# wayveai/fiery

Hardware: NVIDIA H100
Metric: camera->BEV lift frames/sec (6-cam 224x480 -> 200x200) (higher is better)
Workload: dtype f32

## Files before the change

fiery_b200/csrc/common.cuh:

```cuda
#pragma once
#include <cuda.h>
#include <cuda_runtime.h>
#include <cuda_fp16.h>
#include <stdint.h>
#include <stdio.h>
#include <stdlib.h>
#include "../../include/fiery_b200.h"

namespace fiery {

int set_error(int code, const char* fmt, ...);

#define FIERY_CUDA_CHECK(expr)                                                                              \
    do {                                                                                                    \
        cudaError_t _e = (expr);                                                                            \
        if (_e != cudaSuccess)                                                                              \
            return ::fiery::set_error(FIERY_E_CUDA, "%s failed: %s (%s:%d)", #expr, cudaGetErrorString(_e), \
                                      __FILE__, __LINE__);                                                  \
    } while (0)

#define FIERY_REQUIRE(cond, ...)                                             \
    do {                                                                     \
        if (!(cond)) return ::fiery::set_error(FIERY_E_INVALID, __VA_ARGS__); \
    } while (0)
// ... 26 lines not shown
        "mbarrier.try_wait.parity.shared::cta.b64 p, [%1], %2;\n\t"
        "selp.u32 %0, 1, 0, p;\n\t}"
        : "=r"(ok)
        : "r"(smem_addr(bar)), "r"(parity)
        : "memory");
    return ok != 0;
}

__device__ __forceinline__ void mbar_wait(uint64_t* bar, uint32_t parity) {
    uint32_t spins = 0;
    while (!mbar_try_wait(bar, parity)) {
        if (++spins > (1u << 24)) __trap();
    }
}

__device__ __forceinline__ void bulk_load_1d(void* dst, const void* src, uint32_t bytes, uint64_t* bar) {
    asm volatile("cp.async.bulk.shared::cluster.global.mbarrier::complete_tx::bytes [%0], [%1], %2, [%3];"
                 ::"r"(smem_addr(dst)), "l"(src), "r"(bytes), "r"(smem_addr(bar)) : "memory");
}

__device__ __forceinline__ void tma_load_3d(void* dst, const CUtensorMap* map, uint64_t* bar, int c0, int c1, int c2) {
    asm volatile(
        "cp.async.bulk.tensor.3d.shared::cluster.global.mbarrier::complete_tx::bytes [%0], [%1, {%3, %4, %5}], [%2];"
        ::"r"(smem_addr(dst)), "l"(reinterpret_cast<uint64_t>(map)), "r"(smem_addr(bar)), "r"(c0), "r"(c1), "r"(c2)
        : "memory");
}

__device__ __forceinline__ void tma_load_4d(void* dst, const CUtensorMap* map, uint64_t* bar, int c0, int c1, int c2, int c3) {
    asm volatile(
        "cp.async.bulk.tensor.4d.shared::cluster.global.mbarrier::complete_tx::bytes [%0], [%1, {%3, %4, %5, %6}], [%2];"
        ::"r"(smem_addr(dst)), "l"(reinterpret_cast<uint64_t>(map)), "r"(smem_addr(bar)), "r"(c0), "r"(c1), "r"(c2), "r"(c3)
        : "memory");
}

__device__ __forceinline__ void tma_store_4d(const CUtensorMap* map, const void* src, int c0, int c1, int c2, int c3) {
    asm volatile("cp.async.bulk.tensor.4d.global.shared::cta.bulk_group [%0, {%2, %3, %4, %5}], [%1];"
                 ::"l"(reinterpret_cast<uint64_t>(map)), "r"(smem_addr(src)), "r"(c0), "r"(c1), "r"(c2), "r"(c3)
                 : "memory");
}

__device__ __forceinline__ void tma_store_commit_and_wait() {
    asm volatile("cp.async.bulk.commit_group;" ::: "memory");
    asm volatile("cp.async.bulk.wait_group.read 0;" ::: "memory");
}

__device__ __forceinline__ void tma_prefetch_desc(const CUtensorMap* map) {
// ... 31 lines not shown
```

fiery_b200/csrc/lift_fwd.cu:

```cuda
#include <atomic>
#include <mutex>

#include "lift_plan.cuh"
#include "warp_sample.cuh"

namespace fiery {

constexpr int FIN_THREADS = 256;
__global__ void __launch_bounds__(FIN_THREADS)
finalize_nchw_kernel(float* __restrict__ accum, unsigned char* __restrict__ flags, float* __restrict__ bev,
                     long long pillars, int blocks_per_frame, int clear_marks) {
    constexpr int C = 64;
    const int frame = blockIdx.x / blocks_per_frame;
    const long long pl = static_cast<long long>(blockIdx.x % blocks_per_frame) * FIN_THREADS + threadIdx.x;
    if (pl >= pillars) return;
    unsigned char* f = flags + static_cast<size_t>(frame) * pillars + pl;
    float4 v[C / 4];
    if (*f) {
        float4* row = reinterpret_cast<float4*>(accum + (static_cast<size_t>(frame) * pillars + pl) * C);
#pragma unroll
        for (int q = 0; q < C / 4; ++q) v[q] = row[q];
#pragma unroll
        for (int q = 0; q < C / 4; ++q) row[q] = make_float4(0.f, 0.f, 0.f, 0.f);
        if (clear_marks) *f = 0;
// ... 2 lines not shown
        for (int q = 0; q < C / 4; ++q) v[q] = make_float4(0.f, 0.f, 0.f, 0.f);
    }
    float* dst = bev + static_cast<size_t>(frame) * C * pillars + pl;
#pragma unroll
    for (int q = 0; q < C / 4; ++q) {
        dst[static_cast<size_t>(4 * q + 0) * pillars] = v[q].x;
        dst[static_cast<size_t>(4 * q + 1) * pillars] = v[q].y;
        dst[static_cast<size_t>(4 * q + 2) * pillars] = v[q].z;
        dst[static_cast<size_t>(4 * q + 3) * pillars] = v[q].w;
    }
}

constexpr int FT_P = 64;
constexpr int FT_THREADS = 256;

__device__ __forceinline__ void bulk_store_1d(void* dst, const void* src, uint32_t bytes) {
    asm volatile("cp.async.bulk.global.shared::cta.bulk_group [%0], [%1], %2;" ::"l"(dst), "r"(smem_addr(src)), "r"(bytes) : "memory");
}
__device__ __forceinline__ void mbar_arrive(uint64_t* bar) {
    asm volatile("mbarrier.arrive.shared::cta.b64 _, [%0];" ::"r"(smem_addr(bar)) : "memory");
}
__device__ __forceinline__ void tma_store_3d(const CUtensorMap* map, const void* src, int c0, int c1, int c2) {
    asm volatile("cp.async.bulk.tensor.3d.global.shared::cta.bulk_group [%0, {%2, %3, %4}], [%1];"
                 ::"l"(reinterpret_cast<uint64_t>(map)), "r"(smem_addr(src)), "r"(c0), "r"(c1), "r"(c2) : "memory");
}

__global__ void __launch_bounds__(FT_THREADS)
finalize_tma_kernel(const __grid_constant__ CUtensorMap bev_map, float* __restrict__ accum, unsigned char* __restrict__ touched,
                    long long pillars, int tiles_per_frame, int frame_out0, int clear_marks) {
    constexpr int C = 64;
    __shared__ __align__(128) float s_in[FT_P * C];
    __shared__ __align__(128) float s_out[C * FT_P];
    __shared__ __align__(16) float s_zero[C];
    __shared__ __align__(8) uint64_t bar;
    __shared__ unsigned char s_flag[FT_P];
    const int tid = threadIdx.x;
    const int frame = blockIdx.x / tiles_per_frame;
    const long long p0 = static_cast<long long>(blockIdx.x % tiles_per_frame) * FT_P;
    if (tid == 0) {
        tma_prefetch_desc(&bev_map);
        mbar_init(&bar, FT_P);
        fence_mbar_init();
    }
    if (tid >= FT_THREADS - C) s_zero[tid - (FT_THREADS - C)] = 0.f;
    __syncthreads();
    float* row = nullptr;
    unsigned char* mark = nullptr;
    if (tid < FT_P) {
        const long long p = p0 + tid;
        unsigned char f = 0;
        if (p < pillars) {
            mark = touched + static_cast<size_t>(frame) * pillars + p;
            f = *mark;
        }
        s_flag[tid] = f;
        if (f) {
            row = accum + (static_cast<size_t>(frame) * pillars + p) * C;
            mbar_arrive_expect_tx(&bar, C * 4);
            bulk_load_1d(s_in + tid * C, row, C * 4, &bar);
        } else {
            mbar_arrive(&bar);
        }
    }
    __syncthreads();
    mbar_wait(&bar, 0);
    {
        const int lane = tid & 31, w = tid >> 5;
        const int pl = (w & 1) * 32 + lane;
        const int chunk0 = ((w >> 1) & 1) * 8;
        const int i0 = (w >> 2) * 4;
        const bool have = s_flag[pl] != 0;
        const float4* src = reinterpret_cast<const float4*>(s_in + pl * C);
        float* dst = s_out + pl;
        const int l7 = lane & 7;
#pragma unroll
        for (int ii = 0; ii < 4; ++ii) {
            const int chunk = chunk0 + ((i0 + ii) ^ l7);
            float4 v = make_float4(0.f, 0.f, 0.f, 0.f);
            if (have) v = src[chunk];
            float* d = dst + chunk * (4 * FT_P);
            d[0] = v.x; d[FT_P] = v.y; d[2 * FT_P] = v.z; d[3 * FT_P] = v.w;
        }
    }
    fence_proxy_async();
    __syncthreads();
    if (tid == 0) tma_store_3d(&bev_map, s_out, static_cast<int>(p0), 0, frame_out0 + frame);
    if (row) {
        bulk_store_1d(row, s_zero, C * 4);
        if (clear_marks) *mark = 0;
    }
    if (tid == 0 || row) tma_store_commit_and_wait();
}

constexpr int FW_P = 64;
constexpr int FW_THREADS = 256;
__global__ void __launch_bounds__(FW_THREADS)
finalize_warp_kernel(const float* __restrict__ accum, const unsigned char* __restrict__ touched, float* __restrict__ bev,
                     long long pillars, int H, int W, int tiles_per_frame, int frame_out0, const float* __restrict__ theta,
                     const unsigned char* __restrict__ copy_mask) {
    constexpr int C = 64;
    __shared__ float s_out[C][FW_P + 1];
    const int tid = threadIdx.x, lane = tid & 31, warp = tid >> 5;
    const int frame = blockIdx.x / tiles_per_frame;
// ... 25 lines not shown
                    b[k] = __ldg(row + 8 + l);
                }
            }
        }
        float4 ra, rb;
#define FIERY_BLEND(f) \
        ra.f = fmaf(w[3], a[3].f, fmaf(w[2], a[2].f, fmaf(w[1], a[1].f, w[0] * a[0].f))); \
        rb.f = fmaf(w[3], b[3].f, fmaf(w[2], b[2].f, fmaf(w[1], b[1].f, w[0] * b[0].f)));
        FIERY_BLEND(x) FIERY_BLEND(y) FIERY_BLEND(z) FIERY_BLEND(w)
#undef FIERY_BLEND
        s_out[4 * l + 0][pxl] = ra.x; s_out[4 * l + 1][pxl] = ra.y; s_out[4 * l + 2][pxl] = ra.z; s_out[4 * l + 3][pxl] = ra.w;
        s_out[32 + 4 * l + 0][pxl] = rb.x; s_out[32 + 4 * l + 1][pxl] = rb.y; s_out[32 + 4 * l + 2][pxl] = rb.z; s_out[32 + 4 * l + 3][pxl] = rb.w;
    }
    __syncthreads();
    float* dst = bev + static_cast<size_t>(gframe) * C * pillars + p0;
#pragma unroll
    for (int cc = 0; cc < C / (FW_THREADS / 32); ++cc) {
        const int c = warp * (C / (FW_THREADS / 32)) + cc;
#pragma unroll
        for (int half = 0; half < 2; ++half) {
            const int px = half * 32 + lane;
            if (p0 + px < pillars) __stcs(dst + static_cast<size_t>(c) * pillars + px, s_out[c][px]);
        }
    }
}

__global__ void __launch_bounds__(256)
clear_touched_kernel(float* __restrict__ accum, unsigned char* __restrict__ touched, long long n_pillars, int clear_marks) {
    const long long p = static_cast<long long>(blockIdx.x) * blockDim.x + threadIdx.x;
    const int lane = threadIdx.x & 31;
    const unsigned char f = p < n_pillars ? touched[p] : 0;
    unsigned m = __ballot_sync(0xffffffffu, f != 0);
    const long long base = p - lane;
    while (m) {
        const int i = __ffs(m) - 1;
        m &= m - 1;
        reinterpret_cast<float2*>(accum + static_cast<size_t>(base + i) * 64)[lane] = make_float2(0.f, 0.f);
    }
    if (f && clear_marks) touched[p] = 0;
}

__global__ void point_indices_kernel(const LiftParams P, int64_t* __restrict__ idx_out, uint8_t* __restrict__ valid_out,
                                     int32_t* __restrict__ pillar_out, long long n_points_total) {
    const long long gid = static_cast<long long>(blockIdx.x) * blockDim.x + threadIdx.x;
    if (gid >= n_points_total) return;
    const int w = static_cast<int>(gid % P.ww);
    long long r = gid / P.ww;
    const int h = static_cast<int>(r % P.hh); r /= P.hh;
    const int d = static_cast<int>(r % P.D); r /= P.D;
    const int cam_flat = static_cast<int>(r);
    CameraTransform T;
    load_camera(P.calib_mode, P.calib_a, P.calib_b, cam_flat, T);
// ... 23 lines not shown
    for (int k = 0; k < 3; ++k) translation[i * 3 + k] = T.t[k];
}

static std::atomic<int> g_max_chunk_frames{0};
void lift_set_max_chunk_frames(int n) { g_max_chunk_frames.store(n > 0 ? n : 0); }

int lift_chunk_frames(const LiftParams& P) {
    const long long per_frame = P.pillars * P.C * 4 + P.pillars;
    long long c = (1ll << 30) / (per_frame > 0 ? per_frame : 1);
    const int forced = g_max_chunk_frames.load();
    if (forced > 0 && forced < c) c = forced;
    if (c > P.n_frames) c = P.n_frames;
    return static_cast<int>(c < 1 ? 1 : c);
}

size_t lift_scratch_bytes(const LiftParams& P) {
    if (P.bev_layout != FIERY_BEV_NCHW || P.n_frames <= 0) return 0;
    const size_t chunk = static_cast<size_t>(lift_chunk_frames(P));
    return chunk * P.pillars * P.C * 4 + ((chunk * P.pillars + 127) & ~static_cast<size_t>(127));
}

int launch_forward_cols(const LiftParams& P, const void* head, cudaStream_t stream);
int encode_bev_map(CUtensorMap* map, float* bev, long long pillars, int channels, int n_frames, int box_pillars);

constexpr int MAX_CHAINS = 4;
struct ChainResources {
    cudaStream_t side[MAX_CHAINS - 1] = {};
    cudaEvent_t fork = nullptr;
    cudaEvent_t done[MAX_CHAINS - 1] = {};
    bool ready = false;
};
static int chain_resources(ChainResources** out) {
    static thread_local ChainResources pool[16];
    int dev = 0;
    FIERY_CUDA_CHECK(cudaGetDevice(&dev));
    FIERY_REQUIRE(dev >= 0 && dev < 16, "device %d out of range for the chain resources", dev);
    ChainResources& r = pool[dev];
    if (!r.ready) {
        for (int i = 0; i < MAX_CHAINS - 1; ++i) {
            FIERY_CUDA_CHECK(cudaStreamCreateWithFlags(&r.side[i], cudaStreamNonBlocking));
            FIERY_CUDA_CHECK(cudaEventCreateWithFlags(&r.done[i], cudaEventDisableTiming));
        }
        FIERY_CUDA_CHECK(cudaEventCreateWithFlags(&r.fork, cudaEventDisableTiming));
        r.ready = true;
    }
    *out = &r;
    return FIERY_OK;
}

#ifdef FIERY_COLS_AB
static int g_max_chains = MAX_CHAINS;
static int g_chain_min_tiles = 132;
#else
constexpr int g_max_chains = MAX_CHAINS;
constexpr int g_chain_min_tiles = 132;
#endif
int lift_forward_groups(const LiftParams& P, int frames_in_chunk) {
    if (P.bev_layout == FIERY_BEV_NHWC) return 1;
    int groups = frames_in_chunk < g_max_chains ? frames_in_chunk : g_max_chains;
    const long long tiles_per_frame = static_cast<long long>(P.n_cameras) * P.n_wtiles;
    while (groups > 1 && (frames_in_chunk / groups) * tiles_per_frame < g_chain_min_tiles) --groups;
    return groups < 1 ? 1 : groups;
}

int lift_forward_launches(const LiftParams& P) {
    if (P.n_frames <= 0) return 0;
    const int per_group = 1 + (P.bev_layout == FIERY_BEV_NCHW ? 1 : 0);
    const int chunk = lift_chunk_frames(P);
    int n = 0;
    for (int f0 = 0; f0 < P.n_frames; f0 += chunk)
        n += per_group * lift_forward_groups(P, (P.n_frames - f0 < chunk) ? P.n_frames - f0 : chunk);
    return n;
}

static thread_local LaunchTimer* g_timer = nullptr;
void lift_set_timer(LaunchTimer* t) { g_timer = t; }
static inline void timer_begin(cudaStream_t st, int kind) {
// ... 16 lines not shown
    FIERY_REQUIRE(P.D >= 1 && P.D <= 48, "depth_bins=%d not supported by this build (1..48)", P.D);
    FIERY_REQUIRE(P.ww % 4 == 0, "feat_w=%d must be a multiple of 4 (TMA row pitch must be 16-byte aligned)", P.ww);
    FIERY_REQUIRE(P.hh <= PLAN_MAX_ROWS, "feat_h=%d not supported by this build (<= %d)", P.hh, PLAN_MAX_ROWS);
    const bool nchw = P.bev_layout == FIERY_BEV_NCHW;
    FIERY_REQUIRE(!warp_theta || nchw, "the warped lift writes the NCHW layout only");
    FIERY_REQUIRE(scratch != nullptr || !nchw, "NCHW output needs the zeroed scratch buffer of fiery_lift_scratch_bytes()");
    int rc = FIERY_OK;
    LiftParams Q = P;
    Q.head_f16 = head_dtype == FIERY_DTYPE_F16 ? head : nullptr;
#ifdef FIERY_COLS_AB
    if (const char* e = getenv("FIERY_CHAINS")) g_max_chains = atoi(e) < MAX_CHAINS ? atoi(e) : MAX_CHAINS;
    if (const char* e = getenv("FIERY_CHAIN_MIN_TILES")) g_chain_min_tiles = atoi(e);
#endif
    const int chunk = lift_chunk_frames(P);
    float* accum = static_cast<float*>(scratch);
    unsigned char* scratch_marks = nchw ? reinterpret_cast<unsigned char*>(accum + static_cast<size_t>(chunk) * P.pillars * P.C) : nullptr;
    const bool tma_pass = P.pillars % 4 == 0;
    CUtensorMap bev_map;
    if (nchw && tma_pass && !warp_theta) {
        rc = encode_bev_map(&bev_map, bev_out, P.pillars, P.C, P.n_frames, FT_P);
        if (rc != FIERY_OK) return rc;
    }
    ChainResources* res = nullptr;
    for (int f0 = 0; f0 < P.n_frames; f0 += chunk) {
        const int nf = (P.n_frames - f0 < chunk) ? P.n_frames - f0 : chunk;
        const int groups = lift_forward_groups(P, nf);
        cudaStream_t chain[MAX_CHAINS] = {stream};
        if (groups > 1) {
            if (!res) {
                rc = chain_resources(&res);
                if (rc != FIERY_OK) return rc;
            }
            for (int g = 1; g < groups; ++g) chain[g] = res->side[g - 1];
            FIERY_CUDA_CHECK(cudaEventRecord(res->fork, stream));
        }
        for (int g = 0; g < groups; ++g) {
            const int s0 = static_cast<int>(static_cast<long long>(nf) * g / groups);
            const int s1 = static_cast<int>(static_cast<long long>(nf) * (g + 1) / groups);
            cudaStream_t st = chain[g];
            if (g > 0) FIERY_CUDA_CHECK(cudaStreamWaitEvent(st, res->fork, 0));
            Q.frame0 = f0 + s0;
            Q.n_frames = s1 - s0;
            unsigned char* marks = nullptr;
            if (plan) {
                const PlanView v = plan_view(plan, P.n_frames, P.n_cameras, P.n_wtiles, P.pillars, Q.frame0);
                Q.plan_tiles = v.tiles;
                Q.touched = nullptr;
                marks = const_cast<unsigned char*>(v.touched);
            } else {
                Q.plan_tiles = nullptr;
                marks = nchw ? scratch_marks + static_cast<size_t>(s0) * P.pillars : nullptr;
                Q.touched = marks;
            }
            Q.accum = nchw ? accum + static_cast<size_t>(s0) * P.pillars * P.C
                           : bev_out + static_cast<size_t>(Q.frame0) * P.pillars * P.C;
            timer_begin(st, 1);
            rc = launch_forward_cols(Q, head, st);
            timer_end(st);
            if (rc != FIERY_OK) return rc;
            if (nchw) {
                timer_begin(st, 2);
                if (warp_theta) {
                    const int tpf = static_cast<int>((P.pillars + FW_P - 1) / FW_P);
                    finalize_warp_kernel<<<static_cast<unsigned>(tpf) * Q.n_frames, FW_THREADS, 0, st>>>(
                        Q.accum, marks, bev_out, P.pillars, P.grid.X, P.grid.Y, tpf, Q.frame0, warp_theta, warp_copy);
                    const long long n = P.pillars * Q.n_frames;
                    clear_touched_kernel<<<static_cast<unsigned>((n + 255) / 256), 256, 0, st>>>(Q.accum, marks, n, plan ? 0 : 1);
                } else if (tma_pass) {
                    const int tpf = static_cast<int>((P.pillars + FT_P - 1) / FT_P);
                    finalize_tma_kernel<<<static_cast<unsigned>(tpf) * Q.n_frames, FT_THREADS, 0, st>>>(bev_map, Q.accum, marks, P.pillars,
                                                                                                     tpf, Q.frame0, plan ? 0 : 1);
                } else {
                    const int bpf = static_cast<int>((P.pillars + FIN_THREADS - 1) / FIN_THREADS);
                    finalize_nchw_kernel<<<static_cast<unsigned>(bpf) * Q.n_frames, FIN_THREADS, 0, st>>>(
                        Q.accum, marks, bev_out + static_cast<size_t>(Q.frame0) * P.C * P.pillars, P.pillars, bpf, plan ? 0 : 1);
                }
                timer_end(st);
                FIERY_CUDA_CHECK(cudaGetLastError());
            }
            if (g > 0) {
                FIERY_CUDA_CHECK(cudaEventRecord(res->done[g - 1], st));
                FIERY_CUDA_CHECK(cudaStreamWaitEvent(stream, res->done[g - 1], 0));
            }
        }
    }
    return FIERY_OK;
}

int launch_point_indices(const LiftParams& P, int64_t* idx_out, uint8_t* valid_out, int32_t* pillar_out, cudaStream_t stream) {
    const long long total = static_cast<long long>(P.n_frames) * P.n_cameras * P.D * P.hh * P.ww;
    if (total == 0) return FIERY_OK;
    const int threads = 256;
    point_indices_kernel<<<static_cast<unsigned>((total + threads - 1) / threads), threads, 0, stream>>>(
        P, idx_out, valid_out, pillar_out, total);
    FIERY_CUDA_CHECK(cudaGetLastError());
    return FIERY_OK;
}
// ... 10 lines not shown
```

fiery_b200/csrc/lift_fwd_cols.cu:

```cuda
#include <string.h>

#include "lift_plan.cuh"

namespace fiery {

constexpr int COLS_DPAD = 48;
constexpr int COLS_NPAIR = COLS_DPAD * WT;
constexpr int COLS_EVS = 33;
constexpr int COLS_PLAN_STAGE = 4096;
constexpr int COLS_RUNS_STAGED = (COLS_PLAN_STAGE - PLAN_OFF_RUNS) / 4;

struct HeadMapsCols {
    CUtensorMap depth;
    CUtensorMap ctx;
};

struct ColsLayout {
    int hh, C;
    int off_bar, off_plan, off_ev, off_prob, off_ctx, off_pillar, total;
    __host__ __device__ ColsLayout(int hh_, int C_, int n_units) : hh(hh_), C(C_) {
        int o = 0;
        off_bar = o;    o += 16;
        off_plan = o;   o += COLS_PLAN_STAGE;
        off_ev = o;     o += n_units * COLS_EVS * 4;
        o = (o + 127) & ~127;
        off_prob = o;   o += hh * COLS_DPAD * WT * 4;
        o = (o + 127) & ~127;
        off_ctx = o;    o += hh * C * WT * 4;
        o = (o + 127) & ~127;
        off_pillar = o; o += hh * COLS_NPAIR * 4;
        total = o;
    }
};

__device__ __forceinline__ void tma_load_5d(void* dst, const CUtensorMap* map, uint64_t* bar, int c0, int c1, int c2, int c3, int c4) {
    asm volatile(
        "cp.async.bulk.tensor.5d.shared::cluster.global.mbarrier::complete_tx::bytes [%0], [%1, {%3, %4, %5, %6, %7}], [%2];"
        ::"r"(smem_addr(dst)), "l"(reinterpret_cast<uint64_t>(map)), "r"(smem_addr(bar)), "r"(c0), "r"(c1), "r"(c2), "r"(c3), "r"(c4)
        : "memory");
}

__device__ __forceinline__ void cp_async_8(void* dst, const void* src) {
    asm volatile("cp.async.ca.shared.global [%0], [%1], 8;" ::"r"(smem_addr(dst)), "l"(src) : "memory");
}

__device__ __forceinline__ void ffma2(unsigned long long& acc, unsigned long long a, unsigned long long b) {
    asm("{\n\t.reg .f32 a0, a1, b0, b1, c0, c1;\n\t"
        "mov.b64 {a0, a1}, %1;\n\tmov.b64 {b0, b1}, %2;\n\tmov.b64 {c0, c1}, %0;\n\t"
        "fma.rn.f32 c0, a0, b0, c0;\n\tfma.rn.f32 c1, a1, b1, c1;\n\t"
        "mov.b64 %0, {c0, c1};\n\t}" : "+l"(acc) : "l"(a), "l"(b));
}

template <int HALF>
// ... 194 lines not shown
                sum += x[k];
            }
            sum += __shfl_xor_sync(0xffffffffu, sum, 4);
            sum += __shfl_xor_sync(0xffffffffu, sum, 8);
            sum += __shfl_xor_sync(0xffffffffu, sum, 16);
            const float inv = __fdiv_rn(1.0f, sum);
#pragma unroll
            for (int k = 0; k < COLS_DPAD / 8; ++k) base[k * 8 * WT] = x[k] * inv;
        } else {
#pragma unroll
            for (int k = 0; k < COLS_DPAD / 8; ++k) base[k * 8 * WT] = (c8 + 8 * k < P.D) ? 1.0f : 0.f;
        }
    }
}

template <int CPL>
__device__ __forceinline__ void red_channels_if(char* dst, const float (&v)[CPL], unsigned bit) {
    if (CPL == 4)
        asm volatile("{\n\t.reg .pred p;\n\tsetp.ne.u32 p, %5, 0;\n\t@p red.global.add.v4.f32 [%0], {%1, %2, %3, %4};\n\t}"
                     :: "l"(dst), "f"(v[0]), "f"(v[1]), "f"(v[CPL > 2 ? 2 : 0]), "f"(v[CPL > 3 ? 3 : 0]), "r"(bit) : "memory");
    else
        asm volatile("{\n\t.reg .pred p;\n\tsetp.ne.u32 p, %3, 0;\n\t@p red.global.add.v2.f32 [%0], {%1, %2};\n\t}"
                     :: "l"(dst), "f"(v[0]), "f"(v[1]), "r"(bit) : "memory");
}

template <int CPL, int DD, int SD, int COL>
__device__ __forceinline__ void flush_slot(unsigned long long (&acc)[CPL][DD][2], unsigned mw, unsigned own, unsigned flush,
                                           const int* plp, char* out) {
    constexpr int j = SD * 4 + COL;
    if (mw & (1u << j)) {
        const unsigned pl = static_cast<unsigned>(plp[j]);
        float v[CPL];
#pragma unroll
        for (int k = 0; k < CPL; ++k) v[k] = __fadd_rn(half_of<COL & 1>(acc[k][SD][COL >> 1]), 0.0f);
        red_channels_if<CPL>(out + static_cast<size_t>(pl) * (64 * 4), v, flush & (1u << j));
        const unsigned keep = ((own >> j) & 1u) - 1u;
#pragma unroll
        for (int k = 0; k < CPL; ++k) clear_half<COL & 1>(acc[k][SD][COL >> 1], keep);
    }
}

template <int CPL, int DD, int SD>
__device__ __forceinline__ void flush_depth(unsigned long long (&acc)[CPL][DD][2], unsigned mw, unsigned own, unsigned flush,
                                            const int* plp, char* out) {
    if (mw & (0xfu << (4 * SD))) {
        flush_slot<CPL, DD, SD, 0>(acc, mw, own, flush, plp, out); flush_slot<CPL, DD, SD, 1>(acc, mw, own, flush, plp, out);
        flush_slot<CPL, DD, SD, 2>(acc, mw, own, flush, plp, out); flush_slot<CPL, DD, SD, 3>(acc, mw, own, flush, plp, out);
    }
    if constexpr (SD + 1 < DD) flush_depth<CPL, DD, SD + 1>(acc, mw, own, flush, plp, out);
}

template <int CPL, int DD, int MINB, int UNR = 2, bool HALF = false, bool PLANNED = false>
__global__ void __launch_bounds__((COLS_DPAD / DD) * (64 / CPL), MINB)
lift_forward_cols_kernel(const __grid_constant__ HeadMapsCols head_maps, const LiftParams P) {
    constexpr int LPU = 64 / CPL;
    constexpr int NU = COLS_DPAD / DD;
    constexpr int NT = NU * LPU;
    constexpr int SLOTS = 4 * DD;
    static_assert(COLS_DPAD % DD == 0 && SLOTS <= 16 && (LPU == 16 || LPU == 32), "unsupported unit shape");
    extern __shared__ __align__(128) unsigned char smem[];
    const ColsLayout L(P.hh, P.C, NU);
    const int wtile = blockIdx.x % P.n_wtiles;
    const int img_local = blockIdx.x / P.n_wtiles;
    const int img = P.frame0 * P.n_cameras + img_local;
    const int frame = img_local / P.n_cameras;
    const int w0 = wtile * WT;
    const int tid = threadIdx.x;
// ... 5 lines not shown
        if (PLANNED) mbar_init(bar + 1, 1);
        if (!HALF) mbar_init(bar, 1);
        fence_mbar_init();
        if (PLANNED) {
            mbar_arrive_expect_tx(bar + 1, COLS_PLAN_STAGE);
            bulk_load_1d(smem + L.off_plan, rec, COLS_PLAN_STAGE, bar + 1);
        }
    }
    if (HALF) {
        issue_half_tile<CPL, NT>(P, L, smem, img, w0);
    } else if (tid == 0) {
        tma_prefetch_desc(&head_maps.depth);
        tma_prefetch_desc(&head_maps.ctx);
        const uint32_t prob_bytes = P.use_depth ? static_cast<uint32_t>(hh * COLS_DPAD * WT * 4) : 0u;
        mbar_arrive_expect_tx(bar, prob_bytes + static_cast<uint32_t>(hh * L.C * WT * 4));
        if (P.use_depth) tma_load_4d(smem + L.off_prob, &head_maps.depth, bar, w0, 0, 0, img);
        tma_load_5d(smem + L.off_ctx, &head_maps.ctx, bar, w0, 0, 0, 0, img);
    }
    {
        unsigned* s_ev = reinterpret_cast<unsigned*>(smem + L.off_ev);
        for (int i = tid; i < NU * COLS_EVS; i += NT) s_ev[i] = 0u;
    }
    if (!PLANNED) {
        float* s_u = reinterpret_cast<float*>(smem + L.off_plan + GEO_OFF_U);
        float* s_v = reinterpret_cast<float*>(smem + L.off_plan + GEO_OFF_V);
        float* s_d = reinterpret_cast<float*>(smem + L.off_plan + GEO_OFF_D);
        if (tid < WT) s_u[tid] = (w0 + tid < P.ww) ? P.fu[w0 + tid] : 0.f;
        if (tid >= 32 && tid < 64) s_v[tid - 32] = P.fv[min(tid - 32, hh - 1)];
        if (tid >= 64 && tid < 64 + COLS_DPAD) s_d[tid - 64] = (tid - 64 < P.D) ? P.fd[tid - 64] : 0.f;
        if (tid == NT - 1) {
            CameraTransform T;
            load_camera(P.calib_mode, P.calib_a, P.calib_b, img, T);
// ... 13 lines not shown
        if (P.grid.pow2[0] && P.grid.pow2[1]) stage_geometry_cols<true, NT, DD>(P, L, smem, w0, touched);
        else stage_geometry_cols<false, NT, DD>(P, L, smem, w0, touched);
    }
    if (HALF) widen_half_tile<NT>(P, L, smem);
    else mbar_wait(bar, 0);
    softmax_cols<NT>(P, L, smem);
    __syncthreads();

    const int unit = tid / LPU;
    const int cl = tid % LPU;
    const float* pp = reinterpret_cast<const float*>(smem + L.off_prob) + unit * DD * WT;
    const float* cp = reinterpret_cast<const float*>(smem + L.off_ctx) + cl * WT;
    const int* plp = reinterpret_cast<const int*>(smem + L.off_pillar) + unit * SLOTS - COLS_NPAIR;
    char* out = reinterpret_cast<char*>(P.accum + static_cast<size_t>(frame) * P.pillars * P.C + cl * CPL);
    const unsigned* evp = reinterpret_cast<const unsigned*>(smem + L.off_ev) + unit * COLS_EVS + 1;

    unsigned long long acc[CPL][DD][2];
#pragma unroll
    for (int k = 0; k < CPL; ++k)
#pragma unroll
        for (int dd = 0; dd < DD; ++dd) acc[k][dd][0] = acc[k][dd][1] = 0ull;

    unsigned own = 0, flush = 0, mw = 0;
#pragma unroll UNR
    for (int h = 0; h < hh; ++h, pp += COLS_DPAD * WT, cp += 64 * WT, plp += COLS_NPAIR, ++evp) {
        const unsigned ev_next = *evp;
        if (mw) flush_depth<CPL, DD, 0>(acc, mw, own, flush, plp, out);
        ulonglong2 dv[DD];
#pragma unroll
        for (int dd = 0; dd < DD; ++dd) dv[dd] = *reinterpret_cast<const ulonglong2*>(pp + dd * WT);
#pragma unroll
        for (int k = 0; k < CPL; ++k) {
            const ulonglong2 c = *reinterpret_cast<const ulonglong2*>(cp + k * LPU * WT);
#pragma unroll
            for (int dd = 0; dd < DD; ++dd) {
                ffma2(acc[k][dd][0], dv[dd].x, c.x);
                ffma2(acc[k][dd][1], dv[dd].y, c.y);
            }
        }
        own = ev_next & ((1u << SLOTS) - 1u);
        flush = ev_next >> SLOTS;
        mw = LPU == 32 ? own : __reduce_or_sync(0xffffffffu, own);
    }
#pragma unroll
    for (int j = 0; j < SLOTS; ++j) {
        const int pl = plp[j];
        float v[CPL];
#pragma unroll
        for (int k = 0; k < CPL; ++k) {
            const unsigned long long a = acc[k][j >> 2][(j & 3) >> 1];
            v[k] = (j & 1) ? half_of<1>(a) : half_of<0>(a);
        }
        red_channels_if<CPL>(out + static_cast<size_t>(static_cast<unsigned>(pl)) * (64 * 4), v, pl >= 0 ? 1u : 0u);
    }
}

int encode_head_maps_cols(HeadMapsCols* maps, const void* head, const LiftParams& P, int channels_per_lane);

template <int CPL, int DD, int MINB, int UNR, bool HALF, bool PLANNED>
static int launch_forward_cols_t(const LiftParams& P, const void* head, cudaStream_t stream) {
    constexpr int NU = COLS_DPAD / DD, NT = NU * (64 / CPL);
    const ColsLayout L(P.hh, P.C, NU);
    static OncePerDevice once;
    int rc = once.run([]() -> int {
        FIERY_CUDA_CHECK(cudaFuncSetAttribute(lift_forward_cols_kernel<CPL, DD, MINB, UNR, HALF, PLANNED>, cudaFuncAttributeMaxDynamicSharedMemorySize, 227 * 1024));
        FIERY_CUDA_CHECK(cudaFuncSetAttribute(lift_forward_cols_kernel<CPL, DD, MINB, UNR, HALF, PLANNED>, cudaFuncAttributePreferredSharedMemoryCarveout,
                                              cudaSharedmemCarveoutMaxShared));
        return FIERY_OK;
    });
    if (rc != FIERY_OK) return rc;
    FIERY_REQUIRE(L.total <= 227 * 1024, "tile needs %d bytes of shared memory", L.total);
    HeadMapsCols maps;
    if (HALF) {
        memset(&maps, 0, sizeof(maps));
        FIERY_REQUIRE(P.head_f16 != nullptr && (reinterpret_cast<uintptr_t>(P.head_f16) & 7) == 0,
                      "half-precision head tensor must be 8-byte aligned");
    } else {
        rc = encode_head_maps_cols(&maps, head, P, CPL);
        if (rc != FIERY_OK) return rc;
    }
    const long long n_tiles = static_cast<long long>(P.n_frames) * P.n_cameras * P.n_wtiles;
    lift_forward_cols_kernel<CPL, DD, MINB, UNR, HALF, PLANNED><<<static_cast<unsigned>(n_tiles), NT, L.total, stream>>>(maps, P);
    FIERY_CUDA_CHECK(cudaGetLastError());
    return FIERY_OK;
}

int launch_forward_cols(const LiftParams& P, const void* head, cudaStream_t stream) {
    FIERY_REQUIRE(P.hh <= 32, "feat_h=%d not supported by this build (<= 32)", P.hh);
    FIERY_REQUIRE(P.C == 64 && P.D <= COLS_DPAD, "column kernel: C=%d D=%d not supported", P.C, P.D);
    const bool planned = P.plan_tiles != nullptr;
    int n_sm = 0, dev = 0;
    FIERY_CUDA_CHECK(cudaGetDevice(&dev));
    FIERY_CUDA_CHECK(cudaDeviceGetAttribute(&n_sm, cudaDevAttrMultiProcessorCount, dev));
    const long long n_tiles = static_cast<long long>(P.n_frames) * P.n_cameras * P.n_wtiles;
    const long long rem = n_tiles % (2ll * n_sm);
    bool dd3 = planned || !(rem > 0 && rem <= n_sm);
#ifdef FIERY_COLS_AB
    if (const char* e = getenv("FIERY_COLS_VARIANT")) dd3 = atoi(e) < 0 ? dd3 : atoi(e) == 2;
#endif
    const bool half = P.head_f16 != nullptr;
    if (planned) {
        if (dd3) return half ? launch_forward_cols_t<2, 3, 2, 2, true, true>(P, head, stream) : launch_forward_cols_t<2, 3, 2, 2, false, true>(P, head, stream);
        return half ? launch_forward_cols_t<2, 2, 2, 1, true, true>(P, head, stream) : launch_forward_cols_t<2, 2, 2, 1, false, true>(P, head, stream);
    }
    if (dd3) return half ? launch_forward_cols_t<2, 3, 2, 2, true, false>(P, head, stream) : launch_forward_cols_t<2, 3, 2, 2, false, false>(P, head, stream);
    return half ? launch_forward_cols_t<2, 2, 2, 1, true, false>(P, head, stream) : launch_forward_cols_t<2, 2, 2, 1, false, false>(P, head, stream);
}

}
```

Before: 59770.

## Add L2 eviction hints and cap concurrent lanes to shrink accumulator scratch

Adds L2 cache-policy hints across the lift pipeline. Head tensor loads and final BEV stores are marked evict_first, while accumulator reductions and reads are marked evict_last so the scratch accumulator stays resident in L2. Frame groups are now multiplexed onto at most two stream lanes, and each lane reuses its own scratch slice, so scratch shrinks enough to fit in L2. Zeroing stores restore normal policy on a lane's final group. The trade-off is less cross-stream concurrency, plus a risk of L2 thrashing if the persisting set is too large.

Result: faster. 69030 (median of 6 runs) (+15.5%).

```diff
diff --git a/fiery_b200/csrc/common.cuh b/fiery_b200/csrc/common.cuh
--- a/fiery_b200/csrc/common.cuh
+++ b/fiery_b200/csrc/common.cuh
@@ -64,9 +64,29 @@
     }
 }
 
+__device__ __forceinline__ uint64_t l2_evict_first() {
+    uint64_t p;
+    asm("createpolicy.fractional.L2::evict_first.b64 %0, 1.0;" : "=l"(p));
+    return p;
+}
+__device__ __forceinline__ uint64_t l2_evict_last() {
+    uint64_t p;
+    asm("createpolicy.fractional.L2::evict_last.b64 %0, 1.0;" : "=l"(p));
+    return p;
+}
+__device__ __forceinline__ uint64_t l2_evict_normal() {
+    uint64_t p;
+    asm("createpolicy.fractional.L2::evict_normal.b64 %0, 1.0;" : "=l"(p));
+    return p;
+}
+
 __device__ __forceinline__ void bulk_load_1d(void* dst, const void* src, uint32_t bytes, uint64_t* bar) {
     asm volatile("cp.async.bulk.shared::cluster.global.mbarrier::complete_tx::bytes [%0], [%1], %2, [%3];"
                  ::"r"(smem_addr(dst)), "l"(src), "r"(bytes), "r"(smem_addr(bar)) : "memory");
+}
+__device__ __forceinline__ void bulk_load_1d(void* dst, const void* src, uint32_t bytes, uint64_t* bar, uint64_t policy) {
+    asm volatile("cp.async.bulk.shared::cluster.global.mbarrier::complete_tx::bytes.L2::cache_hint [%0], [%1], %2, [%3], %4;"
+                 ::"r"(smem_addr(dst)), "l"(src), "r"(bytes), "r"(smem_addr(bar)), "l"(policy) : "memory");
 }
 
 __device__ __forceinline__ void tma_load_3d(void* dst, const CUtensorMap* map, uint64_t* bar, int c0, int c1, int c2) {
@@ -80,6 +100,14 @@
     asm volatile(
         "cp.async.bulk.tensor.4d.shared::cluster.global.mbarrier::complete_tx::bytes [%0], [%1, {%3, %4, %5, %6}], [%2];"
         ::"r"(smem_addr(dst)), "l"(reinterpret_cast<uint64_t>(map)), "r"(smem_addr(bar)), "r"(c0), "r"(c1), "r"(c2), "r"(c3)
+        : "memory");
+}
+__device__ __forceinline__ void tma_load_4d(void* dst, const CUtensorMap* map, uint64_t* bar, int c0, int c1, int c2, int c3,
+                                            uint64_t policy) {
+    asm volatile(
+        "cp.async.bulk.tensor.4d.shared::cluster.global.mbarrier::complete_tx::bytes.L2::cache_hint [%0], [%1, {%3, %4, %5, %6}], [%2], %7;"
+        ::"r"(smem_addr(dst)), "l"(reinterpret_cast<uint64_t>(map)), "r"(smem_addr(bar)), "r"(c0), "r"(c1), "r"(c2), "r"(c3),
+          "l"(policy)
         : "memory");
 }
 
diff --git a/fiery_b200/csrc/lift_fwd.cu b/fiery_b200/csrc/lift_fwd.cu
--- a/fiery_b200/csrc/lift_fwd.cu
+++ b/fiery_b200/csrc/lift_fwd.cu
@@ -40,20 +40,25 @@
 constexpr int FT_P = 64;
 constexpr int FT_THREADS = 256;
 
-__device__ __forceinline__ void bulk_store_1d(void* dst, const void* src, uint32_t bytes) {
-    asm volatile("cp.async.bulk.global.shared::cta.bulk_group [%0], [%1], %2;" ::"l"(dst), "r"(smem_addr(src)), "r"(bytes) : "memory");
+__device__ __forceinline__ void bulk_store_1d(void* dst, const void* src, uint32_t bytes, uint64_t policy) {
+    asm volatile("cp.async.bulk.global.shared::cta.bulk_group.L2::cache_hint [%0], [%1], %2, %3;"
+                 ::"l"(dst), "r"(smem_addr(src)), "r"(bytes), "l"(policy) : "memory");
 }
 __device__ __forceinline__ void mbar_arrive(uint64_t* bar) {
     asm volatile("mbarrier.arrive.shared::cta.b64 _, [%0];" ::"r"(smem_addr(bar)) : "memory");
 }
-__device__ __forceinline__ void tma_store_3d(const CUtensorMap* map, const void* src, int c0, int c1, int c2) {
-    asm volatile("cp.async.bulk.tensor.3d.global.shared::cta.bulk_group [%0, {%2, %3, %4}], [%1];"
-                 ::"l"(reinterpret_cast<uint64_t>(map)), "r"(smem_addr(src)), "r"(c0), "r"(c1), "r"(c2) : "memory");
+__device__ __forceinline__ void tma_store_3d(const CUtensorMap* map, const void* src, int c0, int c1, int c2, uint64_t policy) {
+    asm volatile("cp.async.bulk.tensor.3d.global.shared::cta.bulk_group.L2::cache_hint [%0, {%2, %3, %4}], [%1], %5;"
+                 ::"l"(reinterpret_cast<uint64_t>(map)), "r"(smem_addr(src)), "r"(c0), "r"(c1), "r"(c2), "l"(policy) : "memory");
+}
+
+__device__ __forceinline__ uint64_t l2_restore_policy(int last_in_lane) {
+    return last_in_lane ? l2_evict_normal() : l2_evict_last();
 }
 
 __global__ void __launch_bounds__(FT_THREADS)
 finalize_tma_kernel(const __grid_constant__ CUtensorMap bev_map, float* __restrict__ accum, unsigned char* __restrict__ touched,
-                    long long pillars, int tiles_per_frame, int frame_out0, int clear_marks) {
+                    long long pillars, int tiles_per_frame, int frame_out0, int clear_marks, int last_in_lane) {
     constexpr int C = 64;
     __shared__ __align__(128) float s_in[FT_P * C];
     __shared__ __align__(128) float s_out[C * FT_P];
@@ -83,7 +88,7 @@
         if (f) {
             row = accum + (static_cast<size_t>(frame) * pillars + p) * C;
             mbar_arrive_expect_tx(&bar, C * 4);
-            bulk_load_1d(s_in + tid * C, row, C * 4, &bar);
+            bulk_load_1d(s_in + tid * C, row, C * 4, &bar, l2_evict_last());
         } else {
             mbar_arrive(&bar);
         }
@@ -110,9 +115,9 @@
     }
     fence_proxy_async();
     __syncthreads();
-    if (tid == 0) tma_store_3d(&bev_map, s_out, static_cast<int>(p0), 0, frame_out0 + frame);
+    if (tid == 0) tma_store_3d(&bev_map, s_out, static_cast<int>(p0), 0, frame_out0 + frame, l2_evict_first());
     if (row) {
-        bulk_store_1d(row, s_zero, C * 4);
+        bulk_store_1d(row, s_zero, C * 4, l2_restore_policy(last_in_lane));
         if (clear_marks) *mark = 0;
     }
     if (tid == 0 || row) tma_store_commit_and_wait();
@@ -168,28 +173,34 @@
     }
     __syncthreads();
     float* dst = bev + static_cast<size_t>(gframe) * C * pillars + p0;
+    const uint64_t once = l2_evict_first();
 #pragma unroll
     for (int cc = 0; cc < C / (FW_THREADS / 32); ++cc) {
         const int c = warp * (C / (FW_THREADS / 32)) + cc;
 #pragma unroll
         for (int half = 0; half < 2; ++half) {
             const int px = half * 32 + lane;
-            if (p0 + px < pillars) __stcs(dst + static_cast<size_t>(c) * pillars + px, s_out[c][px]);
+            if (p0 + px < pillars)
+                asm volatile("st.global.L2::cache_hint.f32 [%0], %1, %2;"
+                             ::"l"(dst + static_cast<size_t>(c) * pillars + px), "f"(s_out[c][px]), "l"(once) : "memory");
         }
     }
 }
 
 __global__ void __launch_bounds__(256)
-clear_touched_kernel(float* __restrict__ accum, unsigned char* __restrict__ touched, long long n_pillars, int clear_marks) {
+clear_touched_kernel(float* __restrict__ accum, unsigned char* __restrict__ touched, long long n_pillars, int clear_marks,
+                     int last_in_lane) {
     const long long p = static_cast<long long>(blockIdx.x) * blockDim.x + threadIdx.x;
     const int lane = threadIdx.x & 31;
     const unsigned char f = p < n_pillars ? touched[p] : 0;
     unsigned m = __ballot_sync(0xffffffffu, f != 0);
     const long long base = p - lane;
+    const uint64_t policy = l2_restore_policy(last_in_lane);
     while (m) {
         const int i = __ffs(m) - 1;
         m &= m - 1;
-        reinterpret_cast<float2*>(accum + static_cast<size_t>(base + i) * 64)[lane] = make_float2(0.f, 0.f);
+        asm volatile("st.global.L2::cache_hint.v2.f32 [%0], {%1, %1}, %2;"
+                     ::"l"(accum + static_cast<size_t>(base + i) * 64 + 2 * lane), "f"(0.f), "l"(policy) : "memory");
     }
     if (f && clear_marks) touched[p] = 0;
 }
@@ -243,20 +254,15 @@
     return static_cast<int>(c < 1 ? 1 : c);
 }
 
-size_t lift_scratch_bytes(const LiftParams& P) {
-    if (P.bev_layout != FIERY_BEV_NCHW || P.n_frames <= 0) return 0;
-    const size_t chunk = static_cast<size_t>(lift_chunk_frames(P));
-    return chunk * P.pillars * P.C * 4 + ((chunk * P.pillars + 127) & ~static_cast<size_t>(127));
-}
-
 int launch_forward_cols(const LiftParams& P, const void* head, cudaStream_t stream);
 int encode_bev_map(CUtensorMap* map, float* bev, long long pillars, int channels, int n_frames, int box_pillars);
 
 constexpr int MAX_CHAINS = 4;
+constexpr int MAX_LANES = 2;
 struct ChainResources {
-    cudaStream_t side[MAX_CHAINS - 1] = {};
+    cudaStream_t side[MAX_LANES - 1] = {};
     cudaEvent_t fork = nullptr;
-    cudaEvent_t done[MAX_CHAINS - 1] = {};
+    cudaEvent_t done[MAX_LANES - 1] = {};
     bool ready = false;
 };
 static int chain_resources(ChainResources** out) {
@@ -266,7 +272,7 @@
     FIERY_REQUIRE(dev >= 0 && dev < 16, "device %d out of range for the chain resources", dev);
     ChainResources& r = pool[dev];
     if (!r.ready) {
-        for (int i = 0; i < MAX_CHAINS - 1; ++i) {
+        for (int i = 0; i < MAX_LANES - 1; ++i) {
             FIERY_CUDA_CHECK(cudaStreamCreateWithFlags(&r.side[i], cudaStreamNonBlocking));
             FIERY_CUDA_CHECK(cudaEventCreateWithFlags(&r.done[i], cudaEventDisableTiming));
         }
@@ -290,6 +296,43 @@
     const long long tiles_per_frame = static_cast<long long>(P.n_cameras) * P.n_wtiles;
     while (groups > 1 && (frames_in_chunk / groups) * tiles_per_frame < g_chain_min_tiles) --groups;
     return groups < 1 ? 1 : groups;
+}
+
+struct LaneLayout {
+    int groups, lanes;
+    int frames;
+    int slice0[MAX_LANES];
+};
+static int group_start(int nf, int groups, int g) { return static_cast<int>(static_cast<long long>(nf) * g / groups); }
+static LaneLayout lane_layout(const LiftParams& P, int frames_in_chunk) {
+    LaneLayout L;
+    L.groups = lift_forward_groups(P, frames_in_chunk);
+    L.lanes = L.groups < MAX_LANES ? L.groups : MAX_LANES;
+    L.frames = 0;
+    for (int l = 0; l < L.lanes; ++l) {
+        int largest = 0;
+        for (int g = l; g < L.groups; g += L.lanes) {
+            const int n = group_start(frames_in_chunk, L.groups, g + 1) - group_start(frames_in_chunk, L.groups, g);
+            largest = n > largest ? n : largest;
+        }
+        L.slice0[l] = L.frames;
+        L.frames += largest;
+    }
+    return L;
+}
+
+static int scratch_frames(const LiftParams& P) {
+    const int chunk = lift_chunk_frames(P);
+    const int full = lane_layout(P, chunk).frames;
+    if (P.n_frames % chunk == 0) return full;
+    const int tail = lane_layout(P, P.n_frames % chunk).frames;
+    return tail > full ? tail : full;
+}
+
+size_t lift_scratch_bytes(const LiftParams& P) {
+    if (P.bev_layout != FIERY_BEV_NCHW || P.n_frames <= 0) return 0;
+    const size_t f = static_cast<size_t>(scratch_frames(P));
+    return f * P.pillars * P.C * 4 + ((f * P.pillars + 127) & ~static_cast<size_t>(127));
 }
 
 int lift_forward_launches(const LiftParams& P) {
@@ -336,7 +379,8 @@
 #endif
     const int chunk = lift_chunk_frames(P);
     float* accum = static_cast<float*>(scratch);
-    unsigned char* scratch_marks = nchw ? reinterpret_cast<unsigned char*>(accum + static_cast<size_t>(chunk) * P.pillars * P.C) : nullptr;
+    unsigned char* scratch_marks =
+        nchw ? reinterpret_cast<unsigned char*>(accum + static_cast<size_t>(scratch_frames(P)) * P.pillars * P.C) : nullptr;
     const bool tma_pass = P.pillars % 4 == 0;
     CUtensorMap bev_map;
     if (nchw && tma_pass && !warp_theta) {
@@ -346,21 +390,23 @@
     ChainResources* res = nullptr;
     for (int f0 = 0; f0 < P.n_frames; f0 += chunk) {
         const int nf = (P.n_frames - f0 < chunk) ? P.n_frames - f0 : chunk;
-        const int groups = lift_forward_groups(P, nf);
-        cudaStream_t chain[MAX_CHAINS] = {stream};
-        if (groups > 1) {
+        const LaneLayout lanes = lane_layout(P, nf);
+        cudaStream_t chain[MAX_LANES] = {stream};
+        if (lanes.lanes > 1) {
             if (!res) {
                 rc = chain_resources(&res);
                 if (rc != FIERY_OK) return rc;
             }
-            for (int g = 1; g < groups; ++g) chain[g] = res->side[g - 1];
+            for (int l = 1; l < lanes.lanes; ++l) chain[l] = res->side[l - 1];
             FIERY_CUDA_CHECK(cudaEventRecord(res->fork, stream));
         }
-        for (int g = 0; g < groups; ++g) {
-            const int s0 = static_cast<int>(static_cast<long long>(nf) * g / groups);
-            const int s1 = static_cast<int>(static_cast<long long>(nf) * (g + 1) / groups);
-            cudaStream_t st = chain[g];
-            if (g > 0) FIERY_CUDA_CHECK(cudaStreamWaitEvent(st, res->fork, 0));
+        for (int g = 0; g < lanes.groups; ++g) {
+            const int s0 = group_start(nf, lanes.groups, g), s1 = group_start(nf, lanes.groups, g + 1);
+            const int lane = g % lanes.lanes;
+            const bool last_in_lane = g + lanes.lanes >= lanes.groups;
+            const size_t slice = static_cast<size_t>(lanes.slice0[lane]);
+            cudaStream_t st = chain[lane];
+            if (lane > 0 && g < lanes.lanes) FIERY_CUDA_CHECK(cudaStreamWaitEvent(st, res->fork, 0));
             Q.frame0 = f0 + s0;
             Q.n_frames = s1 - s0;
             unsigned char* marks = nullptr;
@@ -371,10 +417,10 @@
                 marks = const_cast<unsigned char*>(v.touched);
             } else {
                 Q.plan_tiles = nullptr;
-                marks = nchw ? scratch_marks + static_cast<size_t>(s0) * P.pillars : nullptr;
+                marks = nchw ? scratch_marks + slice * P.pillars : nullptr;
                 Q.touched = marks;
             }
-            Q.accum = nchw ? accum + static_cast<size_t>(s0) * P.pillars * P.C
+            Q.accum = nchw ? accum + slice * P.pillars * P.C
                            : bev_out + static_cast<size_t>(Q.frame0) * P.pillars * P.C;
             timer_begin(st, 1);
             rc = launch_forward_cols(Q, head, st);
@@ -387,11 +433,12 @@
                     finalize_warp_kernel<<<static_cast<unsigned>(tpf) * Q.n_frames, FW_THREADS, 0, st>>>(
                         Q.accum, marks, bev_out, P.pillars, P.grid.X, P.grid.Y, tpf, Q.frame0, warp_theta, warp_copy);
                     const long long n = P.pillars * Q.n_frames;
-                    clear_touched_kernel<<<static_cast<unsigned>((n + 255) / 256), 256, 0, st>>>(Q.accum, marks, n, plan ? 0 : 1);
+                    clear_touched_kernel<<<static_cast<unsigned>((n + 255) / 256), 256, 0, st>>>(Q.accum, marks, n, plan ? 0 : 1,
+                                                                                                 last_in_lane ? 1 : 0);
                 } else if (tma_pass) {
                     const int tpf = static_cast<int>((P.pillars + FT_P - 1) / FT_P);
-                    finalize_tma_kernel<<<static_cast<unsigned>(tpf) * Q.n_frames, FT_THREADS, 0, st>>>(bev_map, Q.accum, marks, P.pillars,
-                                                                                                     tpf, Q.frame0, plan ? 0 : 1);
+                    finalize_tma_kernel<<<static_cast<unsigned>(tpf) * Q.n_frames, FT_THREADS, 0, st>>>(
+                        bev_map, Q.accum, marks, P.pillars, tpf, Q.frame0, plan ? 0 : 1, last_in_lane ? 1 : 0);
                 } else {
                     const int bpf = static_cast<int>((P.pillars + FIN_THREADS - 1) / FIN_THREADS);
                     finalize_nchw_kernel<<<static_cast<unsigned>(bpf) * Q.n_frames, FIN_THREADS, 0, st>>>(
@@ -400,9 +447,9 @@
                 timer_end(st);
                 FIERY_CUDA_CHECK(cudaGetLastError());
             }
-            if (g > 0) {
-                FIERY_CUDA_CHECK(cudaEventRecord(res->done[g - 1], st));
-                FIERY_CUDA_CHECK(cudaStreamWaitEvent(stream, res->done[g - 1], 0));
+            if (lane > 0 && last_in_lane) {
+                FIERY_CUDA_CHECK(cudaEventRecord(res->done[lane - 1], st));
+                FIERY_CUDA_CHECK(cudaStreamWaitEvent(stream, res->done[lane - 1], 0));
             }
         }
     }
diff --git a/fiery_b200/csrc/lift_fwd_cols.cu b/fiery_b200/csrc/lift_fwd_cols.cu
--- a/fiery_b200/csrc/lift_fwd_cols.cu
+++ b/fiery_b200/csrc/lift_fwd_cols.cu
@@ -37,6 +37,14 @@
     asm volatile(
         "cp.async.bulk.tensor.5d.shared::cluster.global.mbarrier::complete_tx::bytes [%0], [%1, {%3, %4, %5, %6, %7}], [%2];"
         ::"r"(smem_addr(dst)), "l"(reinterpret_cast<uint64_t>(map)), "r"(smem_addr(bar)), "r"(c0), "r"(c1), "r"(c2), "r"(c3), "r"(c4)
+        : "memory");
+}
+__device__ __forceinline__ void tma_load_5d(void* dst, const CUtensorMap* map, uint64_t* bar, int c0, int c1, int c2, int c3, int c4,
+                                            uint64_t policy) {
+    asm volatile(
+        "cp.async.bulk.tensor.5d.shared::cluster.global.mbarrier::complete_tx::bytes.L2::cache_hint [%0], [%1, {%3, %4, %5, %6, %7}], [%2], %8;"
+        ::"r"(smem_addr(dst)), "l"(reinterpret_cast<uint64_t>(map)), "r"(smem_addr(bar)), "r"(c0), "r"(c1), "r"(c2), "r"(c3), "r"(c4),
+          "l"(policy)
         : "memory");
 }
 
@@ -261,43 +269,49 @@
     }
 }
 
-template <int CPL>
-__device__ __forceinline__ void red_channels_if(char* dst, const float (&v)[CPL], unsigned bit) {
-    if (CPL == 4)
+template <int CPL, bool HINT>
+__device__ __forceinline__ void red_channels_if(char* dst, const float (&v)[CPL], unsigned bit, uint64_t policy) {
+    if (!HINT && CPL == 4)
         asm volatile("{\n\t.reg .pred p;\n\tsetp.ne.u32 p, %5, 0;\n\t@p red.global.add.v4.f32 [%0], {%1, %2, %3, %4};\n\t}"
                      :: "l"(dst), "f"(v[0]), "f"(v[1]), "f"(v[CPL > 2 ? 2 : 0]), "f"(v[CPL > 3 ? 3 : 0]), "r"(bit) : "memory");
-    else
+    else if (!HINT)
         asm volatile("{\n\t.reg .pred p;\n\tsetp.ne.u32 p, %3, 0;\n\t@p red.global.add.v2.f32 [%0], {%1, %2};\n\t}"
                      :: "l"(dst), "f"(v[0]), "f"(v[1]), "r"(bit) : "memory");
-}
-
-template <int CPL, int DD, int SD, int COL>
+    else if (CPL == 4)
+        asm volatile("{\n\t.reg .pred p;\n\tsetp.ne.u32 p, %5, 0;\n\t@p red.global.add.L2::cache_hint.v4.f32 [%0], {%1, %2, %3, %4}, %6;\n\t}"
+                     :: "l"(dst), "f"(v[0]), "f"(v[1]), "f"(v[CPL > 2 ? 2 : 0]), "f"(v[CPL > 3 ? 3 : 0]), "r"(bit), "l"(policy) : "memory");
+    else
+        asm volatile("{\n\t.reg .pred p;\n\tsetp.ne.u32 p, %3, 0;\n\t@p red.global.add.L2::cache_hint.v2.f32 [%0], {%1, %2}, %4;\n\t}"
+                     :: "l"(dst), "f"(v[0]), "f"(v[1]), "r"(bit), "l"(policy) : "memory");
+}
+
+template <int CPL, int DD, int SD, int COL, bool HINT>
 __device__ __forceinline__ void flush_slot(unsigned long long (&acc)[CPL][DD][2], unsigned mw, unsigned own, unsigned flush,
-                                           const int* plp, char* out) {
+                                           const int* plp, char* out, uint64_t policy) {
     constexpr int j = SD * 4 + COL;
     if (mw & (1u << j)) {
         const unsigned pl = static_cast<unsigned>(plp[j]);
         float v[CPL];
 #pragma unroll
         for (int k = 0; k < CPL; ++k) v[k] = __fadd_rn(half_of<COL & 1>(acc[k][SD][COL >> 1]), 0.0f);
-        red_channels_if<CPL>(out + static_cast<size_t>(pl) * (64 * 4), v, flush & (1u << j));
+        red_channels_if<CPL, HINT>(out + static_cast<size_t>(pl) * (64 * 4), v, flush & (1u << j), policy);
         const unsigned keep = ((own >> j) & 1u) - 1u;
 #pragma unroll
         for (int k = 0; k < CPL; ++k) clear_half<COL & 1>(acc[k][SD][COL >> 1], keep);
     }
 }
 
-template <int CPL, int DD, int SD>
+template <int CPL, int DD, int SD, bool HINT>
 __device__ __forceinline__ void flush_depth(unsigned long long (&acc)[CPL][DD][2], unsigned mw, unsigned own, unsigned flush,
-                                            const int* plp, char* out) {
+                                            const int* plp, char* out, uint64_t policy) {
     if (mw & (0xfu << (4 * SD))) {
-        flush_slot<CPL, DD, SD, 0>(acc, mw, own, flush, plp, out); flush_slot<CPL, DD, SD, 1>(acc, mw, own, flush, plp, out);
-        flush_slot<CPL, DD, SD, 2>(acc, mw, own, flush, plp, out); flush_slot<CPL, DD, SD, 3>(acc, mw, own, flush, plp, out);
-    }
-    if constexpr (SD + 1 < DD) flush_depth<CPL, DD, SD + 1>(acc, mw, own, flush, plp, out);
-}
-
-template <int CPL, int DD, int MINB, int UNR = 2, bool HALF = false, bool PLANNED = false>
+        flush_slot<CPL, DD, SD, 0, HINT>(acc, mw, own, flush, plp, out, policy); flush_slot<CPL, DD, SD, 1, HINT>(acc, mw, own, flush, plp, out, policy);
+        flush_slot<CPL, DD, SD, 2, HINT>(acc, mw, own, flush, plp, out, policy); flush_slot<CPL, DD, SD, 3, HINT>(acc, mw, own, flush, plp, out, policy);
+    }
+    if constexpr (SD + 1 < DD) flush_depth<CPL, DD, SD + 1, HINT>(acc, mw, own, flush, plp, out, policy);
+}
+
+template <int CPL, int DD, int MINB, int UNR = 2, bool HALF = false, bool PLANNED = false, bool HINTS = false>
 __global__ void __launch_bounds__((COLS_DPAD / DD) * (64 / CPL), MINB)
 lift_forward_cols_kernel(const __grid_constant__ HeadMapsCols head_maps, const LiftParams P) {
     constexpr int LPU = 64 / CPL;
@@ -333,8 +347,14 @@
         tma_prefetch_desc(&head_maps.ctx);
         const uint32_t prob_bytes = P.use_depth ? static_cast<uint32_t>(hh * COLS_DPAD * WT * 4) : 0u;
         mbar_arrive_expect_tx(bar, prob_bytes + static_cast<uint32_t>(hh * L.C * WT * 4));
-        if (P.use_depth) tma_load_4d(smem + L.off_prob, &head_maps.depth, bar, w0, 0, 0, img);
-        tma_load_5d(smem + L.off_ctx, &head_maps.ctx, bar, w0, 0, 0, 0, img);
+        if (HINTS) {
+            const uint64_t once = l2_evict_first();
+            if (P.use_depth) tma_load_4d(smem + L.off_prob, &head_maps.depth, bar, w0, 0, 0, img, once);
+            tma_load_5d(smem + L.off_ctx, &head_maps.ctx, bar, w0, 0, 0, 0, img, once);
+        } else {
+            if (P.use_depth) tma_load_4d(smem + L.off_prob, &head_maps.depth, bar, w0, 0, 0, img);
+            tma_load_5d(smem + L.off_ctx, &head_maps.ctx, bar, w0, 0, 0, 0, img);
+        }
     }
     {
         unsigned* s_ev = reinterpret_cast<unsigned*>(smem + L.off_ev);
@@ -378,6 +398,7 @@
     const int* plp = reinterpret_cast<const int*>(smem + L.off_pillar) + unit * SLOTS - COLS_NPAIR;
     char* out = reinterpret_cast<char*>(P.accum + static_cast<size_t>(frame) * P.pillars * P.C + cl * CPL);
     const unsigned* evp = reinterpret_cast<const unsigned*>(smem + L.off_ev) + unit * COLS_EVS + 1;
+    const uint64_t keep = HINTS ? l2_evict_last() : 0;
 
     unsigned long long acc[CPL][DD][2];
 #pragma unroll
@@ -389,7 +410,7 @@
 #pragma unroll UNR
     for (int h = 0; h < hh; ++h, pp += COLS_DPAD * WT, cp += 64 * WT, plp += COLS_NPAIR, ++evp) {
         const unsigned ev_next = *evp;
-        if (mw) flush_depth<CPL, DD, 0>(acc, mw, own, flush, plp, out);
+        if (mw) flush_depth<CPL, DD, 0, HINTS>(acc, mw, own, flush, plp, out, keep);
         ulonglong2 dv[DD];
 #pragma unroll
         for (int dd = 0; dd < DD; ++dd) dv[dd] = *reinterpret_cast<const ulonglong2*>(pp + dd * WT);
@@ -415,20 +436,20 @@
             const unsigned long long a = acc[k][j >> 2][(j & 3) >> 1];
             v[k] = (j & 1) ? half_of<1>(a) : half_of<0>(a);
         }
-        red_channels_if<CPL>(out + static_cast<size_t>(static_cast<unsigned>(pl)) * (64 * 4), v, pl >= 0 ? 1u : 0u);
+        red_channels_if<CPL, HINTS>(out + static_cast<size_t>(static_cast<unsigned>(pl)) * (64 * 4), v, pl >= 0 ? 1u : 0u, keep);
     }
 }
 
 int encode_head_maps_cols(HeadMapsCols* maps, const void* head, const LiftParams& P, int channels_per_lane);
 
-template <int CPL, int DD, int MINB, int UNR, bool HALF, bool PLANNED>
+template <int CPL, int DD, int MINB, int UNR, bool HALF, bool PLANNED, bool HINTS>
 static int launch_forward_cols_t(const LiftParams& P, const void* head, cudaStream_t stream) {
     constexpr int NU = COLS_DPAD / DD, NT = NU * (64 / CPL);
     const ColsLayout L(P.hh, P.C, NU);
     static OncePerDevice once;
     int rc = once.run([]() -> int {
-        FIERY_CUDA_CHECK(cudaFuncSetAttribute(lift_forward_cols_kernel<CPL, DD, MINB, UNR, HALF, PLANNED>, cudaFuncAttributeMaxDynamicSharedMemorySize, 227 * 1024));
-        FIERY_CUDA_CHECK(cudaFuncSetAttribute(lift_forward_cols_kernel<CPL, DD, MINB, UNR, HALF, PLANNED>, cudaFuncAttributePreferredSharedMemoryCarveout,
+        FIERY_CUDA_CHECK(cudaFuncSetAttribute(lift_forward_cols_kernel<CPL, DD, MINB, UNR, HALF, PLANNED, HINTS>, cudaFuncAttributeMaxDynamicSharedMemorySize, 227 * 1024));
+        FIERY_CUDA_CHECK(cudaFuncSetAttribute(lift_forward_cols_kernel<CPL, DD, MINB, UNR, HALF, PLANNED, HINTS>, cudaFuncAttributePreferredSharedMemoryCarveout,
                                               cudaSharedmemCarveoutMaxShared));
         return FIERY_OK;
     });
@@ -444,9 +465,15 @@
         if (rc != FIERY_OK) return rc;
     }
     const long long n_tiles = static_cast<long long>(P.n_frames) * P.n_cameras * P.n_wtiles;
-    lift_forward_cols_kernel<CPL, DD, MINB, UNR, HALF, PLANNED><<<static_cast<unsigned>(n_tiles), NT, L.total, stream>>>(maps, P);
+    lift_forward_cols_kernel<CPL, DD, MINB, UNR, HALF, PLANNED, HINTS><<<static_cast<unsigned>(n_tiles), NT, L.total, stream>>>(maps, P);
     FIERY_CUDA_CHECK(cudaGetLastError());
     return FIERY_OK;
+}
+
+template <int DD, int UNR, bool HALF, bool PLANNED>
+static int launch_layout_t(const LiftParams& P, const void* head, cudaStream_t stream) {
+    return P.bev_layout == FIERY_BEV_NCHW ? launch_forward_cols_t<2, DD, 2, UNR, HALF, PLANNED, true>(P, head, stream)
+                                          : launch_forward_cols_t<2, DD, 2, UNR, HALF, PLANNED, false>(P, head, stream);
 }
 
 int launch_forward_cols(const LiftParams& P, const void* head, cudaStream_t stream) {
@@ -464,11 +491,11 @@
 #endif
     const bool half = P.head_f16 != nullptr;
     if (planned) {
-        if (dd3) return half ? launch_forward_cols_t<2, 3, 2, 2, true, true>(P, head, stream) : launch_forward_cols_t<2, 3, 2, 2, false, true>(P, head, stream);
-        return half ? launch_forward_cols_t<2, 2, 2, 1, true, true>(P, head, stream) : launch_forward_cols_t<2, 2, 2, 1, false, true>(P, head, stream);
-    }
-    if (dd3) return half ? launch_forward_cols_t<2, 3, 2, 2, true, false>(P, head, stream) : launch_forward_cols_t<2, 3, 2, 2, false, false>(P, head, stream);
-    return half ? launch_forward_cols_t<2, 2, 2, 1, true, false>(P, head, stream) : launch_forward_cols_t<2, 2, 2, 1, false, false>(P, head, stream);
-}
-
-}
+        if (dd3) return half ? launch_layout_t<3, 2, true, true>(P, head, stream) : launch_layout_t<3, 2, false, true>(P, head, stream);
+        return half ? launch_layout_t<2, 1, true, true>(P, head, stream) : launch_layout_t<2, 1, false, true>(P, head, stream);
+    }
+    if (dd3) return half ? launch_layout_t<3, 2, true, false>(P, head, stream) : launch_layout_t<3, 2, false, false>(P, head, stream);
+    return half ? launch_layout_t<2, 1, true, false>(P, head, stream) : launch_layout_t<2, 1, false, false>(P, head, stream);
+}
+
+}
```
